# axruff/cuda-flow3d

Hardware: AMD Instinct MI355X
Metric: Mvoxels/s full pyramid solve (higher is better)
Workload: dtype f32; 1 GPU; 512^3 synthetic translated-Gaussian float32 pair (BASELINE config 4), full coarse-to-fine pyramid (40 levels x 40 outer x 5 inner, alpha 7.5, median 5^3, Gaussian sigma 2), frames resident in HBM (value = device-resident rate); parallelism=1 GPU

## Files before the change

### cuda-flow3d_amd/csrc/f3d_median.hip

```cpp
#include "f3d_internal.h"

#include <cstdlib>

namespace {

constexpr int kBX = 64;
constexpr int kBY = 4;

__device__ __forceinline__ void cmp_exchange(float& a, float& b)
{
  const float lo = fminf(a, b);
  const float hi = fmaxf(a, b);
  a = lo;
  b = hi;
}

template <int N>
__device__ __forceinline__ void sort_network(float (&v)[N])
{
#pragma unroll
  for (int p = 1; p < N; p <<= 1) {
#pragma unroll
    for (int k = p; k >= 1; k >>= 1) {
#pragma unroll
      for (int j = k % p; j <= N - 1 - k; j += 2 * k) {
#pragma unroll
        for (int i = 0; i <= (k - 1 < N - j - k - 1 ? k - 1 : N - j - k - 1); ++i) {
          if ((i + j) / (2 * p) == (i + j + k) / (2 * p)) cmp_exchange(v[i + j], v[i + j + k]);
        }
      }
    }
  }
}

template <int N>
__device__ __forceinline__ float rank_middle(float (&v)[N])
{
  sort_network(v);
  return v[N / 2];
}

template <int NB>
__device__ __forceinline__ float rank_nb_of_two_sorted(const float* a, const float* b)
{
  float r = a[NB];
#pragma unroll
  for (int i = 1; i <= NB; ++i) r = fminf(r, fmaxf(a[i - 1], b[NB - i]));
  return r;
}

constexpr int kMaxBatch = 3;
struct MedVols {
  const float* in[kMaxBatch];
  float* out[kMaxBatch];
  int zblocks;
};
__device__ __forceinline__ int med_volume(const MedVols& v, int& zb)
{
  int vol = 0;
  zb = static_cast<int>(blockIdx.z);
  while (zb >= v.zblocks) {
    zb -= v.zblocks;
    ++vol;
  }
  return vol;
}

template <int R>
__global__ __launch_bounds__(kBX* kBY) void k_median_net(MedVols mv, F3dGeo g, int zchunk)
{
  int zb;
  const int vol = med_volume(mv, zb);
  const float* __restrict__ in = mv.in[vol];
  float* __restrict__ out = mv.out[vol];
  constexpr int HALF = R / 2;
  constexpr int TW = kBX + 2 * HALF, TH = kBY + 2 * HALF;
  __shared__ float ring[R][TH][TW];
  const int tid = threadIdx.y * kBX + threadIdx.x;
  const int x0 = blockIdx.x * kBX, y0 = blockIdx.y * kBY;
  const int x = x0 + threadIdx.x;
  const int y = y0 + threadIdx.y;
  const int z0 = g.z_lo + zb * zchunk;
  const int z1 = min(z0 + zchunk, g.z_hi);
  const bool owner = x < g.W && y < g.H;

  auto fetch = [&](int zz) {
    const int zm = f3d_clampi(f3d_mir(zz, g.D), 0, g.D - 1);
    float(*dst)[TW] = ring[((zz % R) + R) % R];
    for (int i = tid; i < TW * TH; i += kBX * kBY) {
      const int ty = i / TW, tx = i - ty * TW;
      const int xs = f3d_clampi(f3d_mir(x0 + tx - HALF, g.W), 0, g.W - 1);
      const int ys = f3d_clampi(f3d_mir(y0 + ty - HALF, g.H), 0, g.H - 1);
      dst[ty][tx] = in[f3d_row(g, ys, zm) + xs];
    }
  };
  for (int zz = z0 - HALF; zz < z0 + HALF; ++zz) fetch(zz);
  for (int z = z0; z < z1; ++z) {
    fetch(z + HALF);
    __syncthreads();
    float v[R * R * R];
#pragma unroll
    for (int iz = 0; iz < R; ++iz) {
      const float(*pl)[TW] = ring[(((z + iz - HALF) % R) + R) % R];
#pragma unroll
      for (int iy = 0; iy < R; ++iy)
#pragma unroll
        for (int ix = 0; ix < R; ++ix) v[(iz * R + iy) * R + ix] = pl[threadIdx.y + iy][threadIdx.x + ix];
    }
    const float med = rank_middle<R * R * R>(v);
    if (owner) out[f3d_row(g, y, z) + x] = med;
    __syncthreads();
  }
}

template <int R>
__global__ __launch_bounds__(kBX* kBY) void k_median_pair(MedVols mv, F3dGeo g, int zchunk)
{
  int zb;
  const int vol = med_volume(mv, zb);
  const float* __restrict__ in = mv.in[vol];
  float* __restrict__ out = mv.out[vol];
  constexpr int HALF = R / 2;
  constexpr int TW = kBX + 2 * HALF, TH = kBY + 2 * HALF;
  constexpr int NS = R + 1;
  constexpr int RR = R * R, NSH = (R - 1) * RR, M = (R * R * R - 1) / 2;
  __shared__ float ring[NS][TH][TW];
  const int tid = threadIdx.y * kBX + threadIdx.x;
  const int x0 = blockIdx.x * kBX, y0 = blockIdx.y * kBY;
  const int x = x0 + threadIdx.x;
  const int y = y0 + threadIdx.y;
  const int z0 = g.z_lo + zb * zchunk;
  const int z1 = min(z0 + zchunk, g.z_hi);
  const bool owner = x < g.W && y < g.H;
  const int zz_max = z1 - 1 + HALF;

  auto slot_of = [&](int zz) { return ((zz % NS) + NS) % NS; };
  auto fetch = [&](int zz) {
    const int zm = f3d_clampi(f3d_mir(min(zz, zz_max), g.D), 0, g.D - 1);
    float(*dst)[TW] = ring[slot_of(zz)];
    for (int i = tid; i < TW * TH; i += kBX * kBY) {
      const int ty = i / TW, tx = i - ty * TW;
      const int xs = f3d_clampi(f3d_mir(x0 + tx - HALF, g.W), 0, g.W - 1);
      const int ys = f3d_clampi(f3d_mir(y0 + ty - HALF, g.H), 0, g.H - 1);
      dst[ty][tx] = in[f3d_row(g, ys, zm) + xs];
    }
  };
  auto gather = [&](int zz, float* v) __attribute__((always_inline)) {
    const float(*pl)[TW] = ring[slot_of(zz)];
#pragma unroll
    for (int iy = 0; iy < R; ++iy)
#pragma unroll
      for (int ix = 0; ix < R; ++ix) v[iy * R + ix] = pl[threadIdx.y + iy][threadIdx.x + ix];
  };
  for (int zz = z0 - HALF; zz < z0 + HALF; ++zz) fetch(zz);
  for (int z = z0; z < z1; z += 2) {
    fetch(z + HALF);
    fetch(z + HALF + 1);
    __syncthreads();
    float s[NSH];
#pragma unroll
    for (int iz = 0; iz < R - 1; ++iz) gather(z - HALF + 1 + iz, s + iz * RR);
    sort_network(s);
    float p[RR];
    gather(z - HALF, p);
    sort_network(p);
    const float med_a = rank_nb_of_two_sorted<RR>(s + (M - RR), p);
    gather(z + HALF + 1, p);
    sort_network(p);
    const float med_b = rank_nb_of_two_sorted<RR>(s + (M - RR), p);
    if (owner) {
      out[f3d_row(g, y, z) + x] = med_a;
      if (z + 1 < z1) out[f3d_row(g, y, z + 1) + x] = med_b;
    }
    __syncthreads();
  }
}

#include "f3d_median_nets.h"

__global__ __launch_bounds__(kBX* kBY) void k_median_keep(MedVols mv, F3dGeo g, int zchunk)
{
  int zb;
  const int vol = med_volume(mv, zb);
  const float* __restrict__ in = mv.in[vol];
  float* __restrict__ out = mv.out[vol];
  constexpr int R = 5, HALF = 2;
  constexpr int TW = kBX + 2 * HALF, TH = kBY + 2 * HALF;
  constexpr int NS = R + 1;
  __shared__ float ring[NS][TH][TW];
  const int tid = threadIdx.y * kBX + threadIdx.x;
  const int x0 = blockIdx.x * kBX, y0 = blockIdx.y * kBY;
  const int x = x0 + threadIdx.x;
  const int y = y0 + threadIdx.y;
  const int z0 = g.z_lo + zb * zchunk;
  const int z1 = min(z0 + zchunk, g.z_hi);
  const bool owner = x < g.W && y < g.H;
  const int zz_max = z1 - 1 + HALF;

  auto slot_of = [&](int zz) { return ((zz % NS) + NS) % NS; };
  auto fetch = [&](int zz) {
    const int zm = f3d_clampi(f3d_mir(min(zz, zz_max), g.D), 0, g.D - 1);
    float(*dst)[TW] = ring[slot_of(zz)];
    for (int i = tid; i < TW * TH; i += kBX * kBY) {
      const int ty = i / TW, tx = i - ty * TW;
      const int xs = f3d_clampi(f3d_mir(x0 + tx - HALF, g.W), 0, g.W - 1);
      const int ys = f3d_clampi(f3d_mir(y0 + ty - HALF, g.H), 0, g.H - 1);
      dst[ty][tx] = in[f3d_row(g, ys, zm) + xs];
    }
  };
  auto sorted_plane = [&](int zz, float (&v)[25]) __attribute__((always_inline)) {
    const float(*pl)[TW] = ring[slot_of(zz)];
#pragma unroll
    for (int iy = 0; iy < R; ++iy)
#pragma unroll
      for (int ix = 0; ix < R; ++ix) v[iy * R + ix] = pl[threadIdx.y + iy][threadIdx.x + ix];
    sort_network(v);
  };
  auto step = [&](const float (&q0)[25], const float (&q1)[25], const float (&q2)[25], const float (&q3)[25], float (&q4)[25],
                  float (&q5)[25], int z) __attribute__((always_inline)) {
    fetch(z + HALF);
    fetch(z + HALF + 1);
    __syncthreads();
    sorted_plane(z + HALF, q4);
    float c[26];
    {
      float ab[50], cd[50];
      merge25(q1, q2, ab);
      merge25(q3, q4, cd);
      candidates(ab, cd, c);
    }
    const float med_a = rank_nb_of_two_sorted<25>(c, q0);
    sorted_plane(z + HALF + 1, q5);
    const float med_b = rank_nb_of_two_sorted<25>(c, q5);
    if (owner) {
      out[f3d_row(g, y, z) + x] = med_a;
      if (z + 1 < z1) out[f3d_row(g, y, z + 1) + x] = med_b;
    }
    __syncthreads();
  };
  float L0[25], L1[25], L2[25], L3[25], L4[25], L5[25];
  for (int zz = z0 - HALF; zz < z0 + HALF; ++zz) fetch(zz);
  __syncthreads();
  sorted_plane(z0 - 2, L0);
  sorted_plane(z0 - 1, L1);
  sorted_plane(z0, L2);
  sorted_plane(z0 + 1, L3);
  for (int z = z0; z < z1; z += 6) {
    step(L0, L1, L2, L3, L4, L5, z);
    if (z + 2 >= z1) break;
    step(L2, L3, L4, L5, L0, L1, z + 2);
    if (z + 4 >= z1) break;
    step(L4, L5, L0, L1, L2, L3, z + 4);
  }
}

__device__ __forceinline__ unsigned order_key(float f)
{
  const unsigned b = __float_as_uint(f);
  return b ^ ((b >> 31) ? 0xFFFFFFFFu : 0x80000000u);
}

template <int R>
__global__ __launch_bounds__(kBX* kBY) void k_median_bisect(MedVols mv, F3dGeo g)
{
  int zb;
  const int vol = med_volume(mv, zb);
  const float* __restrict__ in = mv.in[vol];
  float* __restrict__ out = mv.out[vol];
  constexpr int HALF = R / 2;
  constexpr int RANK = (R * R * R) / 2;
  const int x = blockIdx.x * kBX + threadIdx.x;
  const int y = blockIdx.y * kBY + threadIdx.y;
  const int z = g.z_lo + zb;
  if (x >= g.W || y >= g.H) return;
  int xs[R];
#pragma unroll
  for (int i = 0; i < R; ++i) xs[i] = f3d_mir(x + i - HALF, g.W);
  unsigned prefix = 0;
  for (int bit = 31; bit >= 0; --bit) {
    const unsigned cand = prefix | (1u << bit);
    int below = 0;
    for (int iz = 0; iz < R; ++iz) {
      const int zz = f3d_mir(z + iz - HALF, g.D);
      for (int iy = 0; iy < R; ++iy) {
        const size_t row = f3d_row(g, f3d_mir(y + iy - HALF, g.H), zz);
#pragma unroll
        for (int ix = 0; ix < R; ++ix) below += order_key(in[row + xs[ix]]) < cand ? 1 : 0;
      }
    }
    if (below <= RANK) prefix = cand;
  }
  const unsigned b = (prefix >> 31) ? (prefix ^ 0x80000000u) : ~prefix;
  out[f3d_row(g, y, z) + x] = __uint_as_float(b);
}

}

static int median_launch(const f3d_devptr* inputs, size_t count, size_t width, size_t height, size_t depth, size_t radius,
                         const f3d_devptr* outputs, const f3d_slab* slab, const char* who)
{
  F3D_REQUIRE_READY(who);
  if (!inputs || !outputs) return f3d::fail("%s: null argument", who);
  if (count == 0 || count > static_cast<size_t>(kMaxBatch)) return f3d::fail("%s: %zu volumes (one launch takes 1 .. %d)", who, count, kMaxBatch);
  for (size_t i = 0; i < count; ++i)
    for (size_t j = 0; j < count; ++j)
      if (inputs[i] == outputs[j]) return f3d::fail("%s: input buffer cannot serve as output buffer", who);
  if (radius != 3 && radius != 5 && radius != 7)
    return f3d::fail("%s: wrong median radius (%zu). Supported values: 3, 5, 7", who, radius);
  F3dGeo g;
  if (!f3d::make_geo(&g, width, height, depth, slab, who)) return 1;
  const int half = static_cast<int>(radius) / 2;
  if (g.W <= half || g.H <= half || g.D <= half)
    return f3d::fail("%s: every dimension must exceed radius/2 = %d for the mirror boundary", who, half);
  if (g.z_lo == g.z_hi) return 0;
  {
    const int dc = static_cast<int>(f3d::container().depth);
    int lo = g.z_lo - half < 0 ? 0 : g.z_lo - half;
    int hi = g.z_hi + half > g.D ? g.D : g.z_hi + half;
    if (g.z_lo - half < 0 && half + 1 > hi) hi = half + 1;
    if (g.z_hi + half > g.D && g.D - 1 - half < lo) lo = g.D - 1 - half;
    if (lo < g.z_base || hi - g.z_base > dc)
      return f3d::fail("%s: planes [%d,%d) needed but the container holds [%d,%d)", who, lo, hi, g.z_base, g.z_base + dc);
  }
  const dim3 block(kBX, kBY, 1);
  MedVols mv = {};
  for (size_t i = 0; i < count; ++i) {
    mv.in[i] = f3d_ptr<const float>(inputs[i]);
    mv.out[i] = f3d_ptr<float>(outputs[i]);
  }
  const unsigned nvol = static_cast<unsigned>(count);
  if (count > 1 && static_cast<long>(g.z_hi - g.z_lo) * static_cast<long>(count) > 65535L) {
    for (size_t i = 0; i < count; ++i)
      if (int e = median_launch(inputs + i, 1, width, height, depth, radius, outputs + i, slab, who)) return e;
    return 0;
  }
  if (radius == 7) {
    mv.zblocks = g.z_hi - g.z_lo;
    const dim3 grid((g.W + kBX - 1) / kBX, (g.H + kBY - 1) / kBY, mv.zblocks * nvol);
    hipLaunchKernelGGL(k_median_bisect<7>, grid, block, 0, f3d::stream(), mv, g);
  } else {
    const int planes = g.z_hi - g.z_lo;
    const long tiles = static_cast<long>((g.W + kBX - 1) / kBX) * ((g.H + kBY - 1) / kBY) * static_cast<long>(count);
    const char* forced_env = std::getenv("F3D_MEDIAN_PAIR");
    const int forced = forced_env ? std::atoi(forced_env) : -1;
    if (forced == 0) {
      long nz = (8192 + tiles - 1) / tiles;
      if (nz > planes) nz = planes;
      if (nz < 1) nz = 1;
      const int zchunk = static_cast<int>((planes + nz - 1) / nz);
      mv.zblocks = (planes + zchunk - 1) / zchunk;
      const dim3 grid((g.W + kBX - 1) / kBX, (g.H + kBY - 1) / kBY, mv.zblocks * nvol);
      if (radius == 3) hipLaunchKernelGGL(k_median_net<3>, grid, block, 0, f3d::stream(), mv, g, zchunk);
      if (radius == 5) hipLaunchKernelGGL(k_median_net<5>, grid, block, 0, f3d::stream(), mv, g, zchunk);
    } else {
      const bool can_keep = radius == 5 && forced != 1;
      const bool can_pair = !(radius == 5 && forced == 2);
      const long pair_ops = radius == 5 ? 2600 : 330;
      int zchunk = 2;
      bool keep = false;
      long best = -1;
      for (int zc = 2; zc <= planes + 1; zc += 2) {
        const long wgs = tiles * ((planes + zc - 1) / zc);
        const long rounds = (wgs + 255) / 256, thin = wgs < 512 ? 13 : 10;
        const long cost_pair = rounds * thin * (300 + (zc / 2) * pair_ops);
        const long cost_keep = rounds * thin * (300 + 1200 + (zc / 2) * 1430);
        if (can_pair && (best < 0 || cost_pair < best)) {
          best = cost_pair;
          zchunk = zc;
          keep = false;
        }
        if (can_keep && (best < 0 || cost_keep < best)) {
          best = cost_keep;
          zchunk = zc;
          keep = true;
        }
      }
      mv.zblocks = (planes + zchunk - 1) / zchunk;
      const dim3 grid((g.W + kBX - 1) / kBX, (g.H + kBY - 1) / kBY, mv.zblocks * nvol);
      if (radius == 3) hipLaunchKernelGGL(k_median_pair<3>, grid, block, 0, f3d::stream(), mv, g, zchunk);
      if (radius == 5 && keep) hipLaunchKernelGGL(k_median_keep, grid, block, 0, f3d::stream(), mv, g, zchunk);
      if (radius == 5 && !keep) hipLaunchKernelGGL(k_median_pair<5>, grid, block, 0, f3d::stream(), mv, g, zchunk);
    }
  }
  F3D_HIP(hipGetLastError());
  return 0;
}

extern "C" int f3d_median(f3d_devptr input, size_t width, size_t height, size_t depth, size_t radius, f3d_devptr output,
                          const f3d_slab* slab)
{
  return median_launch(&input, 1, width, height, depth, radius, &output, slab, "f3d_median");
}

extern "C" int f3d_median_n(const f3d_devptr* inputs, size_t count, size_t width, size_t height, size_t depth, size_t radius,
                            const f3d_devptr* outputs, const f3d_slab* slab)
{
  return median_launch(inputs, count, width, height, depth, radius, outputs, slab, "f3d_median_n");
}
```

Before: 71.17 Mvoxels/s.

## Add shared-column 5^3 median kernel with LDS DMA ring and sorted column reuse

```diff
diff --git a/cuda-flow3d_amd/csrc/f3d_median.hip b/cuda-flow3d_amd/csrc/f3d_median.hip
--- a/cuda-flow3d_amd/csrc/f3d_median.hip
+++ b/cuda-flow3d_amd/csrc/f3d_median.hip
@@ -251,6 +251,140 @@
     step(L2, L3, L4, L5, L0, L1, z + 2);
     if (z + 4 >= z1) break;
     step(L4, L5, L0, L1, L2, L3, z + 4);
+  }
+}
+
+#include "f3d_median_nets_share.h"
+
+typedef __attribute__((address_space(3))) float LdsFloat;
+__device__ __forceinline__ void dma4_lane(const float* lane_addr, float* lds_dst)
+{
+  const unsigned m0v = static_cast<unsigned>(reinterpret_cast<unsigned long>((LdsFloat*)lds_dst));
+  asm volatile("s_nop 0\n\tglobal_load_lds_dword %0, off" ::"v"(lane_addr), "{m0}"(m0v) : "memory");
+}
+
+__global__ __launch_bounds__(kBX* kBY) void k_median_share(MedVols mv, F3dGeo g, int zchunk)
+{
+  int zb;
+  const int vol = med_volume(mv, zb);
+  const float* __restrict__ in = mv.in[vol];
+  float* __restrict__ out = mv.out[vol];
+  constexpr int HALF = 2;
+  constexpr int TW = kBX + 2 * HALF, TH = kBY + 2 * HALF;
+  constexpr int NT = kBX * kBY, NCOL = TW * kBY;
+  __shared__ float keep[50][NT];
+  __shared__ float ring[2][TH][TW];
+  __shared__ float cols[2][5][NCOL];
+  const int tid = threadIdx.y * kBX + threadIdx.x;
+  const int x0 = blockIdx.x * kBX, y0 = blockIdx.y * kBY;
+  const int x = x0 + threadIdx.x;
+  const int y = y0 + threadIdx.y;
+  const int z0 = g.z_lo + zb * zchunk;
+  const int z1 = min(z0 + zchunk, g.z_hi);
+  const bool owner = x < g.W && y < g.H;
+  const int zz_max = z1 - 1 + HALF;
+  const int own = threadIdx.y * TW + threadIdx.x;
+
+  static_assert(kBX == 64, "one row of the workgroup must be one wave");
+  constexpr int NF = (TW * TH + NT - 1) / NT;
+  const int wave = __builtin_amdgcn_readfirstlane(static_cast<int>(threadIdx.y));
+  int off[NF];
+#pragma unroll
+  for (int k = 0; k < NF; ++k) {
+    const int i = min(tid + k * NT, TW * TH - 1);
+    const int ty = i / TW, tx = i - ty * TW;
+    const int xs = f3d_clampi(f3d_mir(x0 + tx - HALF, g.W), 0, g.W - 1);
+    const int ys = f3d_clampi(f3d_mir(y0 + ty - HALF, g.H), 0, g.H - 1);
+    off[k] = ys * g.pitch + xs;
+  }
+  auto request = [&](int zz, int slot) __attribute__((always_inline)) {
+    const int zm = f3d_clampi(f3d_mir(min(zz, zz_max), g.D), 0, g.D - 1);
+    const float* plane = in + f3d_row(g, 0, zm);
+    float* dst = &ring[slot][0][0] + wave * 64;
+#pragma unroll
+    for (int k = 0; k < NF; ++k)
+      if (tid + k * NT < TW * TH) dma4_lane(plane + off[k], dst + k * NT);
+  };
+  auto sort_column = [&](int slot, int c) __attribute__((always_inline)) {
+    const float* top = &ring[slot][0][0] + c;
+    float raw[5], s[5];
+#pragma unroll
+    for (int k = 0; k < 5; ++k) raw[k] = top[k * TW];
+    sort5(raw, s);
+#pragma unroll
+    for (int k = 0; k < 5; ++k) cols[slot][k][c] = s[k];
+  };
+  auto columns = [&]() __attribute__((always_inline)) {
+    asm volatile("s_waitcnt vmcnt(0)" ::: "memory");
+    __syncthreads();
+#pragma unroll
+    for (int slot = 0; slot < 2; ++slot) {
+      sort_column(slot, tid);
+      if (tid < NCOL - NT) sort_column(slot, NT + tid);
+    }
+    __syncthreads();
+  };
+  auto plane_list = [&](int slot, float (&q)[25]) __attribute__((always_inline)) {
+    float v[25];
+#pragma unroll
+    for (int j = 0; j < 5; ++j)
+#pragma unroll
+      for (int k = 0; k < 5; ++k) v[j * 5 + k] = cols[slot][k][own + j];
+    merge5x5(v, q);
+  };
+  auto step = [&](float (&la)[25], const float (&lb)[25], const float (&lc)[25], float (&q4)[25], int z) __attribute__((always_inline)) {
+    columns();
+    if (z + 2 < z1) {
+      request(z + HALF + 2, 0);
+      request(z + HALF + 3, 1);
+    }
+    plane_list(0, q4);
+    float c[26];
+    {
+      float ab[50], cd[50];
+      merge25(lc, q4, cd);
+#pragma unroll
+      for (int i = 0; i < 50; ++i) ab[i] = keep[i][tid];
+      candidates(ab, cd, c);
+#pragma unroll
+      for (int i = 0; i < 50; ++i) keep[i][tid] = cd[i];
+    }
+    const float med_a = rank_nb_of_two_sorted<25>(c, la);
+    plane_list(1, la);
+    const float med_b = rank_nb_of_two_sorted<25>(c, la);
+    if (owner) {
+      out[f3d_row(g, y, z) + x] = med_a;
+      if (z + 1 < z1) out[f3d_row(g, y, z + 1) + x] = med_b;
+    }
+    (void)lb;
+  };
+  float A[25], B[25], C[25], E[25];
+  request(z0 - 2, 0);
+  request(z0 - 1, 1);
+  columns();
+  request(z0, 0);
+  request(z0 + 1, 1);
+  plane_list(0, A);
+  plane_list(1, E);
+  columns();
+  request(z0 + 2, 0);
+  request(z0 + 3, 1);
+  plane_list(0, B);
+  plane_list(1, C);
+  {
+    float ab[50];
+    merge25(E, B, ab);
+#pragma unroll
+    for (int i = 0; i < 50; ++i) keep[i][tid] = ab[i];
+  }
+  for (int z = z0; z < z1; z += 8) {
+    step(A, B, C, E, z);
+    if (z + 2 >= z1) break;
+    step(B, E, A, C, z + 2);
+    if (z + 4 >= z1) break;
+    step(E, C, B, A, z + 4);
+    if (z + 6 >= z1) break;
+    step(C, A, E, B, z + 6);
   }
 }
 
@@ -353,9 +487,11 @@
       if (radius == 3) hipLaunchKernelGGL(k_median_net<3>, grid, block, 0, f3d::stream(), mv, g, zchunk);
       if (radius == 5) hipLaunchKernelGGL(k_median_net<5>, grid, block, 0, f3d::stream(), mv, g, zchunk);
     } else {
+      const bool share = radius == 5 && forced != 1 && forced != 2;
       const bool can_keep = radius == 5 && forced != 1;
-      const bool can_pair = !(radius == 5 && forced == 2);
+      const bool can_pair = !(radius == 5 && (forced == 2 || forced == 3));
       const long pair_ops = radius == 5 ? 2600 : 330;
+      const long keep_ops = share ? 1010 : 1430, keep_start = share ? 1190 : 1200;
       int zchunk = 2;
       bool keep = false;
       long best = -1;
@@ -363,7 +499,7 @@
         const long wgs = tiles * ((planes + zc - 1) / zc);
         const long rounds = (wgs + 255) / 256, thin = wgs < 512 ? 13 : 10;
         const long cost_pair = rounds * thin * (300 + (zc / 2) * pair_ops);
-        const long cost_keep = rounds * thin * (300 + 1200 + (zc / 2) * 1430);
+        const long cost_keep = rounds * thin * (300 + keep_start + (zc / 2) * keep_ops);
         if (can_pair && (best < 0 || cost_pair < best)) {
           best = cost_pair;
           zchunk = zc;
@@ -378,7 +514,8 @@
       mv.zblocks = (planes + zchunk - 1) / zchunk;
       const dim3 grid((g.W + kBX - 1) / kBX, (g.H + kBY - 1) / kBY, mv.zblocks * nvol);
       if (radius == 3) hipLaunchKernelGGL(k_median_pair<3>, grid, block, 0, f3d::stream(), mv, g, zchunk);
-      if (radius == 5 && keep) hipLaunchKernelGGL(k_median_keep, grid, block, 0, f3d::stream(), mv, g, zchunk);
+      if (radius == 5 && keep && share) hipLaunchKernelGGL(k_median_share, grid, block, 0, f3d::stream(), mv, g, zchunk);
+      if (radius == 5 && keep && !share) hipLaunchKernelGGL(k_median_keep, grid, block, 0, f3d::stream(), mv, g, zchunk);
       if (radius == 5 && !keep) hipLaunchKernelGGL(k_median_pair<5>, grid, block, 0, f3d::stream(), mv, g, zchunk);
     }
   }
diff --git a/cuda-flow3d_amd/csrc/f3d_median_nets_share.h b/cuda-flow3d_amd/csrc/f3d_median_nets_share.h
--- /dev/null
+++ b/cuda-flow3d_amd/csrc/f3d_median_nets_share.h
@@ -0,0 +1,262 @@
+#ifndef F3D_MEDIAN_NETS_SHARE_H_
+#define F3D_MEDIAN_NETS_SHARE_H_
+
+__device__ __forceinline__ void sort5(const float (&v)[5], float (&out)[5])
+{
+  const float t0 = fminf(v[0], v[1]);
+  const float t1 = fmaxf(v[0], v[1]);
+  const float t2 = fminf(v[3], v[4]);
+  const float t3 = fmaxf(v[3], v[4]);
+  const float t4 = fminf(v[2], t2);
+  const float t5 = fmaxf(v[2], t2);
+  const float t6 = fminf(t5, t3);
+  const float t7 = fmaxf(t5, t3);
+  const float t8 = fminf(t0, t4);
+  const float t9 = fmaxf(t0, t4);
+  const float t10 = fminf(t9, t7);
+  const float t11 = fmaxf(t9, t7);
+  const float t12 = fminf(t1, t6);
+  const float t13 = fmaxf(t1, t6);
+  const float t14 = fminf(t10, t12);
+  const float t15 = fmaxf(t10, t12);
+  const float t16 = fminf(t11, t13);
+  const float t17 = fmaxf(t11, t13);
+  out[0] = t8;
+  out[1] = t14;
+  out[2] = t15;
+  out[3] = t16;
+  out[4] = t17;
+}
+
+__device__ __forceinline__ void merge5x5(const float (&v)[25], float (&out)[25])
+{
+  const float t0 = fminf(v[0], v[5]);
+  const float t1 = fmaxf(v[0], v[5]);
+  const float t2 = fminf(v[4], v[9]);
+  const float t3 = fmaxf(v[4], v[9]);
+  const float t4 = fminf(t1, t2);
+  const float t5 = fmaxf(t1, t2);
+  const float t6 = fminf(v[2], v[7]);
+  const float t7 = fmaxf(v[2], v[7]);
+  const float t8 = fminf(t4, t6);
+  const float t9 = fmaxf(t4, t6);
+  const float t10 = fminf(t5, t7);
+  const float t11 = fmaxf(t5, t7);
+  const float t12 = fminf(v[1], v[6]);
+  const float t13 = fmaxf(v[1], v[6]);
+  const float t14 = fminf(v[3], v[8]);
+  const float t15 = fmaxf(v[3], v[8]);
+  const float t16 = fminf(t13, t14);
+  const float t17 = fmaxf(t13, t14);
+  const float t18 = fminf(t8, t12);
+  const float t19 = fmaxf(t8, t12);
+  const float t20 = fminf(t9, t16);
+  const float t21 = fmaxf(t9, t16);
+  const float t22 = fminf(t10, t17);
+  const float t23 = fmaxf(t10, t17);
+  const float t24 = fminf(t11, t15);
+  const float t25 = fmaxf(t11, t15);
+  const float t26 = fminf(v[10], v[15]);
+  const float t27 = fmaxf(v[10], v[15]);
+  const float t28 = fminf(v[14], v[19]);
+  const float t29 = fmaxf(v[14], v[19]);
+  const float t30 = fminf(t27, t28);
+  const float t31 = fmaxf(t27, t28);
+  const float t32 = fminf(v[12], v[17]);
+  const float t33 = fmaxf(v[12], v[17]);
+  const float t34 = fminf(t30, t32);
+  const float t35 = fmaxf(t30, t32);
+  const float t36 = fminf(t31, t33);
+  const float t37 = fmaxf(t31, t33);
+  const float t38 = fminf(v[11], v[16]);
+  const float t39 = fmaxf(v[11], v[16]);
+  const float t40 = fminf(v[13], v[18]);
+  const float t41 = fmaxf(v[13], v[18]);
+  const float t42 = fminf(t39, t40);
+  const float t43 = fmaxf(t39, t40);
+  const float t44 = fminf(t34, t38);
+  const float t45 = fmaxf(t34, t38);
+  const float t46 = fminf(t35, t42);
+  const float t47 = fmaxf(t35, t42);
+  const float t48 = fminf(t36, t43);
+  const float t49 = fmaxf(t36, t43);
+  const float t50 = fminf(t37, t41);
+  const float t51 = fmaxf(t37, t41);
+  const float t52 = fminf(t26, v[20]);
+  const float t53 = fmaxf(t26, v[20]);
+  const float t54 = fminf(t53, t51);
+  const float t55 = fmaxf(t53, t51);
+  const float t56 = fminf(t47, v[24]);
+  const float t57 = fmaxf(t47, v[24]);
+  const float t58 = fminf(t54, t56);
+  const float t59 = fmaxf(t54, t56);
+  const float t60 = fminf(t55, t57);
+  const float t61 = fmaxf(t55, t57);
+  const float t62 = fminf(t45, v[22]);
+  const float t63 = fmaxf(t45, v[22]);
+  const float t64 = fminf(t63, t49);
+  const float t65 = fmaxf(t63, t49);
+  const float t66 = fminf(t58, t62);
+  const float t67 = fmaxf(t58, t62);
+  const float t68 = fminf(t59, t64);
+  const float t69 = fmaxf(t59, t64);
+  const float t70 = fminf(t60, t65);
+  const float t71 = fmaxf(t60, t65);
+  const float t72 = fminf(t44, v[21]);
+  const float t73 = fmaxf(t44, v[21]);
+  const float t74 = fminf(t73, t29);
+  const float t75 = fmaxf(t73, t29);
+  const float t76 = fminf(t74, t48);
+  const float t77 = fmaxf(t74, t48);
+  const float t78 = fminf(t46, v[23]);
+  const float t79 = fmaxf(t46, v[23]);
+  const float t80 = fminf(t79, t50);
+  const float t81 = fmaxf(t79, t50);
+  const float t82 = fminf(t76, t78);
+  const float t83 = fmaxf(t76, t78);
+  const float t84 = fminf(t77, t80);
+  const float t85 = fmaxf(t77, t80);
+  const float t86 = fminf(t75, t81);
+  const float t87 = fmaxf(t75, t81);
+  const float t88 = fminf(t66, t72);
+  const float t89 = fmaxf(t66, t72);
+  const float t90 = fminf(t67, t82);
+  const float t91 = fmaxf(t67, t82);
+  const float t92 = fminf(t68, t83);
+  const float t93 = fmaxf(t68, t83);
+  const float t94 = fminf(t69, t84);
+  const float t95 = fmaxf(t69, t84);
+  const float t96 = fminf(t70, t85);
+  const float t97 = fmaxf(t70, t85);
+  const float t98 = fminf(t71, t86);
+  const float t99 = fmaxf(t71, t86);
+  const float t100 = fminf(t61, t87);
+  const float t101 = fmaxf(t61, t87);
+  const float t102 = fminf(t0, t52);
+  const float t103 = fmaxf(t0, t52);
+  const float t104 = fminf(t25, t95);
+  const float t105 = fmaxf(t25, t95);
+  const float t106 = fminf(t103, t104);
+  const float t107 = fmaxf(t103, t104);
+  const float t108 = fminf(t21, t91);
+  const float t109 = fmaxf(t21, t91);
+  const float t110 = fminf(t109, t99);
+  const float t111 = fmaxf(t109, t99);
+  const float t112 = fminf(t106, t108);
+  const float t113 = fmaxf(t106, t108);
+  const float t114 = fminf(t107, t110);
+  const float t115 = fmaxf(t107, t110);
+  const float t116 = fminf(t105, t111);
+  const float t117 = fmaxf(t105, t111);
+  const float t118 = fminf(t19, t89);
+  const float t119 = fmaxf(t19, t89);
+  const float t120 = fminf(t119, t97);
+  const float t121 = fmaxf(t119, t97);
+  const float t122 = fminf(t23, t93);
+  const float t123 = fmaxf(t23, t93);
+  const float t124 = fminf(t123, t101);
+  const float t125 = fmaxf(t123, t101);
+  const float t126 = fminf(t120, t122);
+  const float t127 = fmaxf(t120, t122);
+  const float t128 = fminf(t121, t124);
+  const float t129 = fmaxf(t121, t124);
+  const float t130 = fminf(t112, t118);
+  const float t131 = fmaxf(t112, t118);
+  const float t132 = fminf(t113, t126);
+  const float t133 = fmaxf(t113, t126);
+  const float t134 = fminf(t114, t127);
+  const float t135 = fmaxf(t114, t127);
+  const float t136 = fminf(t115, t128);
+  const float t137 = fmaxf(t115, t128);
+  const float t138 = fminf(t116, t129);
+  const float t139 = fmaxf(t116, t129);
+  const float t140 = fminf(t117, t125);
+  const float t141 = fmaxf(t117, t125);
+  const float t142 = fminf(t18, t88);
+  const float t143 = fmaxf(t18, t88);
+  const float t144 = fminf(t3, t96);
+  const float t145 = fmaxf(t3, t96);
+  const float t146 = fminf(t143, t144);
+  const float t147 = fmaxf(t143, t144);
+  const float t148 = fminf(t22, t92);
+  const float t149 = fmaxf(t22, t92);
+  const float t150 = fminf(t149, t100);
+  const float t151 = fmaxf(t149, t100);
+  const float t152 = fminf(t146, t148);
+  const float t153 = fmaxf(t146, t148);
+  const float t154 = fminf(t147, t150);
+  const float t155 = fmaxf(t147, t150);
+  const float t156 = fminf(t145, t151);
+  const float t157 = fmaxf(t145, t151);
+  const float t158 = fminf(t20, t90);
+  const float t159 = fmaxf(t20, t90);
+  const float t160 = fminf(t159, t98);
+  const float t161 = fmaxf(t159, t98);
+  const float t162 = fminf(t24, t94);
+  const float t163 = fmaxf(t24, t94);
+  const float t164 = fminf(t160, t162);
+  const float t165 = fmaxf(t160, t162);
+  const float t166 = fminf(t161, t163);
+  const float t167 = fmaxf(t161, t163);
+  const float t168 = fminf(t152, t158);
+  const float t169 = fmaxf(t152, t158);
+  const float t170 = fminf(t153, t164);
+  const float t171 = fmaxf(t153, t164);
+  const float t172 = fminf(t154, t165);
+  const float t173 = fmaxf(t154, t165);
+  const float t174 = fminf(t155, t166);
+  const float t175 = fmaxf(t155, t166);
+  const float t176 = fminf(t156, t167);
+  const float t177 = fmaxf(t156, t167);
+  const float t178 = fminf(t130, t142);
+  const float t179 = fmaxf(t130, t142);
+  const float t180 = fminf(t131, t168);
+  const float t181 = fmaxf(t131, t168);
+  const float t182 = fminf(t132, t169);
+  const float t183 = fmaxf(t132, t169);
+  const float t184 = fminf(t133, t170);
+  const float t185 = fmaxf(t133, t170);
+  const float t186 = fminf(t134, t171);
+  const float t187 = fmaxf(t134, t171);
+  const float t188 = fminf(t135, t172);
+  const float t189 = fmaxf(t135, t172);
+  const float t190 = fminf(t136, t173);
+  const float t191 = fmaxf(t136, t173);
+  const float t192 = fminf(t137, t174);
+  const float t193 = fmaxf(t137, t174);
+  const float t194 = fminf(t138, t175);
+  const float t195 = fmaxf(t138, t175);
+  const float t196 = fminf(t139, t176);
+  const float t197 = fmaxf(t139, t176);
+  const float t198 = fminf(t140, t177);
+  const float t199 = fmaxf(t140, t177);
+  const float t200 = fminf(t141, t157);
+  const float t201 = fmaxf(t141, t157);
+  out[0] = t102;
+  out[1] = t178;
+  out[2] = t179;
+  out[3] = t180;
+  out[4] = t181;
+  out[5] = t182;
+  out[6] = t183;
+  out[7] = t184;
+  out[8] = t185;
+  out[9] = t186;
+  out[10] = t187;
+  out[11] = t188;
+  out[12] = t189;
+  out[13] = t190;
+  out[14] = t191;
+  out[15] = t192;
+  out[16] = t193;
+  out[17] = t194;
+  out[18] = t195;
+  out[19] = t196;
+  out[20] = t197;
+  out[21] = t198;
+  out[22] = t199;
+  out[23] = t200;
+  out[24] = t201;
+}
+
+#endif
```

Measured after the change: 72.42 Mvoxels/s (median of 6 runs). +1.8%, better.
